# az16/MD_RDM

Measured on AMD Instinct MI355X. Metric: depth-maps/sec NYU 228x304 batch=16 fwd+bwd, higher is better.
Workload: dtype f32 (bf16x6-split 1x1 forward of dense_e2/e3, bf16x3-split gradient GEMMs of dense_e2/e3/e4); 1 GPU; NYU-v2 228x304 batch=16/GPU full train step (fwd+losses+bwd+AdamW), DepthEstimationNet 90.5M params; global_batch=16, parallelism=dp1

## Files before the change

md_rdm_amd/csrc/xsplit.hip:

```cpp
#include <algorithm>
#include <stdlib.h>

#include "rdm_common.h"
#include "elementwise.h"
#include "xsplit.h"
#include "xsplit_dev.h"

namespace rdm {

namespace {

__device__ __forceinline__ bf16x8 tr_frag(const unsigned char* base0, const unsigned char* base1, int imm) {
#if defined(__HIP_DEVICE_COMPILE__)
  typedef s16x4 __attribute__((address_space(3))) * lds_s16x4;
  const s16x4 a = __builtin_amdgcn_ds_read_tr16_b64_v4i16((lds_s16x4)(base0 + imm));
  const s16x4 b = __builtin_amdgcn_ds_read_tr16_b64_v4i16((lds_s16x4)(base1 + imm));
  const s16x8 ab = {a.x, a.y, a.z, a.w, b.x, b.y, b.z, b.w};
  return __builtin_bit_cast(bf16x8, ab);
#else
  return bf16x8{};
#endif
}

struct XsWgradArgs {
// ... 290 lines not shown
          const int idx = b0 + u * 256 + ts, slot = idx / 12, quad = idx - slot * 12;
          if (idx < total4) {
            u32x2 hi, lo;
            split4(v[u][0], v[u][1], v[u][2], v[u][3], hi, lo);
            *reinterpret_cast<u32x2*>(Ahi + (slot + 1) * XD_SLOT + quad * 8) = hi;
            if (NP == 3) *reinterpret_cast<u32x2*>(Alo + (slot + 1) * XD_SLOT + quad * 8) = lo;
          }
        }
      }
      if (ts < 24) *reinterpret_cast<u32x2*>(xs_smem + (ts % 12) * 8 + (ts / 12) * p.plane_bytes) = u32x2{0u, 0u};
      base0 = ((ts & 15) + W + 1 + 1) * XD_SLOT - 32768;
#pragma unroll
      for (int i = 0; i < XD_MT; ++i) {
        const int m = m0 + i * 16 + (ts & 15);
        const bool ok = m < p.M;
        const int b = m / HW, rem = m - b * HW, y = rem / W, x = rem - y * W;
        int v = 0;
#pragma unroll
        for (int tap = 0; tap < 9; ++tap) {
          const int r = tap / 3, q = tap - 3 * r;
          const bool valid = ok && (unsigned)(y + 1 - r) < (unsigned)p.H && (unsigned)(x + 1 - q) < (unsigned)W;
          v |= valid ? (1 << tap) : 0;
        }
        if (i % 3 == 0) vm[i / 3] = v; else vm[i / 3] |= v << (10 * (i % 3));
      }
      __syncthreads();
    }
    const int ct16 = tile * (XD_BN / 16) + 2 * wave;
    if (ct16 * 16 >= p.Cb) continue;
    int ln = lane;
    asm volatile("" : "+v"(ln));
    const int l16 = ln & 15, g = ln >> 4, hi2 = g >> 1;
    const unsigned wv = (unsigned)(ln * 16);
    asm volatile("" : "+v"(base0));
#pragma unroll
    for (int q = 0; q < XD_KSTEPS / 2; ++q) asm volatile("" : "+v"(dpk[q]));
    f32x4 acc[XD_MT][2];
#pragma unroll
    for (int i = 0; i < XD_MT; ++i) { acc[i][0] = f32x4{0.f, 0.f, 0.f, 0.f}; acc[i][1] = f32x4{0.f, 0.f, 0.f, 0.f}; }
    bf16x8 wf[2][2][2];
    auto load_w = [&](int j, bf16x8 (&w)[2][2]) {
#pragma unroll
      for (int t = 0; t < 2; ++t)
#pragma unroll
        for (int pl = 0; pl < (NP == 3 ? 2 : 1); ++pl)
          w[t][pl] = __builtin_bit_cast(bf16x8, __builtin_amdgcn_raw_buffer_load_b128(srdW, (int)(wv + (unsigned)((ct16 + t) * (XD_KSTEPS * 2048))), j * 2048 + pl * 1024, 0));
    };
    const bool t1ok = (ct16 + 1) * 16 < p.Cb;
    f32x4 xv[XD_EA + 1][XD_EC][2];
    f32x4 xs[2] = {{0.f, 0.f, 0.f, 0.f}, {0.f, 0.f, 0.f, 0.f}}, xt[2] = {{0.f, 0.f, 0.f, 0.f}, {0.f, 0.f, 0.f, 0.f}};
    const int c40 = ct16 * 16 + 4 * g;
    int ml = m0 + l16;
    const unsigned vx0 = (unsigned)ml * (unsigned)(p.ldx * 4) + (unsigned)(c40 * 4);
    const int osz = (NP == 1 && p.out_bf16) ? 2 : 4;
    const unsigned vo0 = (unsigned)ml * (unsigned)(p.ldc * osz) + (unsigned)(c40 * osz);
    auto gate_load = [&](int c) {
#pragma unroll
      for (int u = 0; u < XD_EC; ++u)
#pragma unroll
        for (int t = 0; t < 2; ++t) {
          const int i = c * XD_EC + u;
          xv[c % (XD_EA + 1)][u][t] = __builtin_bit_cast(f32x4, __builtin_amdgcn_raw_buffer_load_b128(srdX, (int)(((t == 0 || t1ok) && ml + i * 16 < p.M) ? vx0 + 64u * t : OOB), i * 16 * p.ldx * 4, 0));
        }
    };
    load_w(0, wf[0]);
    bf16x8 gq[2][2];
    auto frag = [&](int j, int i, bf16x8 (&f)[2]) {
      const int dj = (int)((dpk[j >> 1] >> ((j & 1) * 16)) & 0xFFFFu);
      const int tapj = (4 * j) / 6 + (((4 * j) % 6 == 4) ? hi2 : 0);
      const int a = (base0 + i * (16 * XD_SLOT) + dj) & __builtin_amdgcn_sbfe(vm[i / 3], (unsigned)(tapj + 10 * (i % 3)), 1u);
      f[0] = *reinterpret_cast<const bf16x8*>(Ahi + a);
      if (NP == 3) f[1] = *reinterpret_cast<const bf16x8*>(Alo + a);
    };
    frag(0, 0, gq[0]);
#pragma unroll
    for (int j = 0; j < XD_KSTEPS; ++j) {
      if (j + 1 < XD_KSTEPS) load_w(j + 1, wf[(j + 1) & 1]);
      if (MASK && j >= XD_KSTEPS - XD_EK) gate_load(j - (XD_KSTEPS - XD_EK));
#pragma unroll
      for (int i = 0; i < XD_MT; ++i) {
        const int cur = (j * XD_MT + i) & 1;
        if (i + 1 < XD_MT) frag(j, i + 1, gq[cur ^ 1]);
        else if (j + 1 < XD_KSTEPS) frag(j + 1, 0, gq[cur ^ 1]);
        __builtin_amdgcn_sched_barrier(0);
#pragma unroll
        for (int t = 0; t < 2; ++t) {
          if (NP == 3) {
            acc[i][t] = __builtin_amdgcn_mfma_f32_16x16x32_bf16(wf[j & 1][t][1], gq[cur][0], acc[i][t], 0, 0, 0);
            acc[i][t] = __builtin_amdgcn_mfma_f32_16x16x32_bf16(wf[j & 1][t][0], gq[cur][1], acc[i][t], 0, 0, 0);
          }
          acc[i][t] = __builtin_amdgcn_mfma_f32_16x16x32_bf16(wf[j & 1][t][0], gq[cur][0], acc[i][t], 0, 0, 0);
        }
        __builtin_amdgcn_sched_barrier(0);
      }
    }

    f32x4 s0[2] = {{0.f, 0.f, 0.f, 0.f}, {0.f, 0.f, 0.f, 0.f}}, s1[2] = {{0.f, 0.f, 0.f, 0.f}, {0.f, 0.f, 0.f, 0.f}};
    if (MASK) {
#pragma unroll
      for (int t = 0; t < 2; ++t)
        if (t == 0 || t1ok) { xs[t] = *reinterpret_cast<const f32x4*>(p.x_scale + c40 + 16 * t); xt[t] = *reinterpret_cast<const f32x4*>(p.x_shift + c40 + 16 * t); }
#pragma unroll
      for (int c = XD_EK; c < XD_EA; ++c) gate_load(c);
    }
#pragma unroll
    for (int c = 0; c < XD_NCH; ++c) {
      if (MASK && c + XD_EA < XD_NCH) { gate_load(c + XD_EA); __builtin_amdgcn_sched_barrier(0); }
#pragma unroll
      for (int u = 0; u < XD_EC; ++u)
#pragma unroll
        for (int t = 0; t < 2; ++t) {
          const int i = c * XD_EC + u;
          const bool ok = (t == 0 || t1ok) && ml + i * 16 < p.M;
          unsigned char* const orow = reinterpret_cast<unsigned char*>(p.out) + ((long)i * 16 * p.ldc + 16 * t) * osz;
          f32x4 v = acc[i][t];
          if (MASK) {
            const f32x4 x = xv[c % (XD_EA + 1)][u][t];
#pragma unroll
            for (int e = 0; e < 4; ++e) v[e] = fmaf(x[e], xs[t][e], xt[t][e]) > 0.f ? v[e] : 0.f;
            if (ok) { s0[t] += v; s1[t] += v * x; }
          }
          if (NP == 1 && p.out_bf16) {
            const bf16x2 lo2 = {(__bf16)v[0], (__bf16)v[1]}, hi2 = {(__bf16)v[2], (__bf16)v[3]};
            if (ok) *reinterpret_cast<u32x2*>(orow + vo0) = u32x2{__builtin_bit_cast(unsigned, lo2), __builtin_bit_cast(unsigned, hi2)};
          } else if (ok) *reinterpret_cast<f32x4*>(orow + vo0) = v;
        }
    }
    if (MASK) {
      const int sl = 4 * g + l16;
#pragma unroll
      for (int t = 0; t < 2; ++t) {
        const int c4 = ct16 * 16 + 16 * t + sl;
#pragma unroll
        for (int e = 0; e < 4; ++e) {
          float a = s0[t][e], b = s1[t][e];
          a += __shfl_xor(a, 1); b += __shfl_xor(b, 1);
          a += __shfl_xor(a, 2); b += __shfl_xor(b, 2);
          a += __shfl_xor(a, 4); b += __shfl_xor(b, 4);
          a += __shfl_xor(a, 8); b += __shfl_xor(b, 8);
          if (l16 == e) { s0[t][0] = a; s1[t][0] = b; }
        }
        if (l16 < 4 && (t == 0 || t1ok)) {
          atomicAdd(p.stat0 + c4, (double)s0[t][0]);
          atomicAdd(p.stat1 + c4, (double)s1[t][0]);
        }
      }
    }
  }
}


constexpr int X1_MTW_BIG = 5, X1_MTW_SMALL = 2, X1_NTW = 6, X1_BNMAX = 2 * X1_NTW * 16;
constexpr int X1_W_IMG = X1_BNMAX * 64;
constexpr int x1_lds(int mtw) { return 2 * (2 * (4 * mtw * 16 * 64) + 2 * X1_W_IMG); }

struct XsDgrad1Args {
  const float* G; int ldg; int K;
  int g_bf16;
  int g_split;
  int acc;
  const unsigned char* Wp;
  float* out; int ldc;
  const float* X; int ldx; const float* x_scale; const float* x_shift;
  double* stat0; double* stat1;
  int M, C, ksteps;
  int PT;
  int mtiles, ctiles;
  int ct_c0[12], ct_n[12];
  unsigned g_bytes, w_bytes, x_bytes;
};

__global__ __launch_bounds__(256) void k_xs_pack_w1_dgrad(const float* __restrict__ w, int ldw, int K, int C, int ksteps, unsigned char* __restrict__ Wp) {
  const long idx = (long)blockIdx.x * 256 + threadIdx.x;
  const int c = (int)(idx % C);
  const long r1 = idx / C;
  const int ch = (int)(r1 & 3), j = (int)(r1 >> 2);
  if (j >= ksteps) return;
  float v[8];
#pragma unroll
  for (int e = 0; e < 8; ++e) {
    const int k = 32 * j + 8 * ch + e;
    v[e] = k < K ? w[(long)k * ldw + c] : 0.f;
  }
  u32x2 h0, l0, h1, l1;
  split4(v[0], v[1], v[2], v[3], h0, l0);
  split4(v[4], v[5], v[6], v[7], h1, l1);
  const int chs = ch ^ (((c >> 2) & 1) << 1);
  const long plane = (long)ksteps * C * 64;
  unsigned char* dst = Wp + ((long)j * C + c) * 64 + chs * 16;
  *reinterpret_cast<u32x4*>(dst) = u32x4{h0[0], h0[1], h1[0], h1[1]};
  *reinterpret_cast<u32x4*>(dst + plane) = u32x4{l0[0], l0[1], l1[0], l1[1]};
}

template <bool MASK, int NP, int MTW, int D>
__global__ __launch_bounds__(512, 2) void xs_dgrad1x1_kernel(XsDgrad1Args p) {
  constexpr int X1_MTW = MTW, X1_G_IMG = 4 * MTW * 16 * 64, X1_STAGE = 2 * X1_G_IMG + 2 * X1_W_IMG;
  extern __shared__ __attribute__((aligned(1024))) unsigned char x1_smem[];
  const int tid = threadIdx.x, lane = tid & 63, wave = __builtin_amdgcn_readfirstlane(tid >> 6);
  const int l16 = lane & 15, g = lane >> 4;
  const int wc = wave & 1, wp = wave >> 1;
  const unsigned total = gridDim.x, L = blockIdx.x, xq = L & 7u, qq = total >> 3, rr = total & 7u;
  const unsigned item = xq * qq + (xq < rr ? xq : rr) + (L >> 3);
  const int mt = (int)(item / (unsigned)p.ctiles), ctile = (int)(item - (unsigned)mt * (unsigned)p.ctiles);
  const int BM = p.PT * 16, m0 = mt * BM;
  const int nct = p.ct_n[ctile], ct0 = p.ct_c0[ctile], BN = nct * 16;
  const int ntw_max = (nct + 1) >> 1, tw0 = wc * ntw_max, ntw = min(ntw_max, nct - tw0);
  const int npw_max = (p.PT + 3) >> 2, pw0 = wp * npw_max, npw = max(0, min(npw_max, p.PT - pw0));
  const __amdgpu_buffer_rsrc_t srdG = make_srd(p.G, p.g_bytes), srdW = make_srd(p.Wp, p.w_bytes), srdX = make_srd(p.X, p.x_bytes);

  unsigned g_voff[X1_MTW]; unsigned g_lds[X1_MTW]; int g_k[X1_MTW];
#pragma unroll
  for (int u = 0; u < X1_MTW; ++u) {
    const int idx = tid + 512 * u, row = idx >> 3, f4 = idx & 7;
    const bool ok = row < BM && m0 + row < p.M;
    g_k[u] = ok ? 4 * f4 : 0x40000000;
    g_voff[u] = (NP == 1 && p.g_bf16) ? (unsigned)(m0 + row) * (unsigned)(p.ldg * 2) + (unsigned)(f4 * 8)
                                      : (unsigned)(m0 + row) * (unsigned)(p.ldg * 4) + (unsigned)(f4 * 16);
    g_lds[u] = (unsigned)(row * 64 + (((f4 >> 1) ^ (((row >> 2) & 1) << 1)) * 16) + (f4 & 1) * 8);
  }
  const int wpieces = BN * 8;
  const unsigned w_plane = (unsigned)p.ksteps * (unsigned)p.C * 64u;
  f32x4 rg[D][X1_MTW]; u32x4 rw[D][3];
  auto load_slab = [&](int set, int j) {
#pragma unroll
    for (int u = 0; u < X1_MTW; ++u) {
      if (NP == 1 && p.g_bf16) {
        const u32x2 h = __builtin_amdgcn_raw_buffer_load_b64(srdG, (int)((32 * j + g_k[u] < p.K) ? g_voff[u] + (unsigned)(j * 64) : OOB), 0, 0);
        rg[set][u] = f32x4{__uint_as_float(h[0]), __uint_as_float(h[1]), 0.f, 0.f};
      } else {
        rg[set][u] = __builtin_bit_cast(f32x4, __builtin_amdgcn_raw_buffer_load_b128(srdG, (int)((32 * j + g_k[u] < p.K) ? g_voff[u] + (unsigned)(j * 128) : OOB), 0, 0));
      }
    }
#pragma unroll
    for (int u = 0; u < 3; ++u) {
      const int q = tid + 512 * u, pl = q >= BN * 4, r = pl ? q - BN * 4 : q;
      rw[set][u] = __builtin_amdgcn_raw_buffer_load_b128(srdW, (int)((q < wpieces && j < p.ksteps) ? (unsigned)pl * w_plane + ((unsigned)j * (unsigned)p.C + (unsigned)(ct0 * 16)) * 64u + (unsigned)r * 16u : OOB), 0, 0);
    }
  };
  auto store_slab = [&](int set, unsigned char* st) {
#pragma unroll
    for (int u = 0; u < X1_MTW; ++u) {
      if ((tid + 512 * u) >> 3 < BM) {
        u32x2 hi, lo;
        if (NP == 1 && p.g_bf16) hi = u32x2{__float_as_uint(rg[set][u][0]), __float_as_uint(rg[set][u][1])};
        else if (NP == 3 && p.g_split) { hi = u32x2{__float_as_uint(rg[set][u][0]), __float_as_uint(rg[set][u][1])}; lo = u32x2{__float_as_uint(rg[set][u][2]), __float_as_uint(rg[set][u][3])}; }
        else split4(rg[set][u][0], rg[set][u][1], rg[set][u][2], rg[set][u][3], hi, lo);
        *reinterpret_cast<u32x2*>(st + g_lds[u]) = hi;
        if (NP == 3) *reinterpret_cast<u32x2*>(st + X1_G_IMG + g_lds[u]) = lo;
      }
    }
#pragma unroll
    for (int u = 0; u < 3; ++u) {
      const int q = tid + 512 * u, pl = q >= BN * 4, r = pl ? q - BN * 4 : q;
      if (q < wpieces) *reinterpret_cast<u32x4*>(st + 2 * X1_G_IMG + pl * X1_W_IMG + r * 16) = rw[set][u];
    }
  };

  f32x4 acc[X1_MTW][X1_NTW];
#pragma unroll
  for (int i = 0; i < X1_MTW; ++i)
#pragma unroll
    for (int t = 0; t < X1_NTW; ++t) acc[i][t] = f32x4{0.f, 0.f, 0.f, 0.f};
  const unsigned fr = (unsigned)(l16 * 64 + ((g ^ (((l16 >> 2) & 1) << 1)) * 16));

  load_slab(0, 0);
  store_slab(0, x1_smem);
#pragma unroll
  for (int d = 1; d < D; ++d) load_slab(d, d);
  __syncthreads();
  const int ksteps_pad = (p.ksteps + D - 1) / D * D;
  for (int j0 = 0; j0 < ksteps_pad; j0 += D) {
#pragma unroll
    for (int u = 0; u < D; ++u) {
      const int j = j0 + u;
      const bool more = j + 1 < ksteps_pad;
      const unsigned char* const st = x1_smem + (j & 1) * X1_STAGE;
      load_slab(u, j + D);
      bf16x8 gh[X1_MTW], gl[X1_MTW];
#pragma unroll
      for (int i = 0; i < X1_MTW; ++i)
        if (i < npw) {
          gh[i] = *reinterpret_cast<const bf16x8*>(st + (pw0 + i) * 1024 + fr);
          gl[i] = *reinterpret_cast<const bf16x8*>(st + X1_G_IMG + (pw0 + i) * 1024 + fr);
        }
#pragma unroll
      for (int t = 0; t < X1_NTW; ++t)
        if (t < ntw) {
          const bf16x8 wh = *reinterpret_cast<const bf16x8*>(st + 2 * X1_G_IMG + (tw0 + t) * 1024 + fr);
          const bf16x8 wl = *reinterpret_cast<const bf16x8*>(st + 2 * X1_G_IMG + X1_W_IMG + (tw0 + t) * 1024 + fr);
#pragma unroll
          for (int i = 0; i < X1_MTW; ++i)
            if (i < npw) {
              if (NP == 3) {
                acc[i][t] = __builtin_amdgcn_mfma_f32_16x16x32_bf16(wl, gh[i], acc[i][t], 0, 0, 0);
                acc[i][t] = __builtin_amdgcn_mfma_f32_16x16x32_bf16(wh, gl[i], acc[i][t], 0, 0, 0);
              }
              acc[i][t] = __builtin_amdgcn_mfma_f32_16x16x32_bf16(wh, gh[i], acc[i][t], 0, 0, 0);
            }
        }
      if (more) store_slab((u + 1) % D, x1_smem + ((j + 1) & 1) * X1_STAGE);
      __syncthreads();
    }
  }

#pragma unroll
  for (int t = 0; t < X1_NTW; ++t) {
    if (t >= ntw) continue;
    const int c4 = (ct0 + tw0 + t) * 16 + 4 * g;
    const bool cok = c4 < p.C;
    f32x4 xs = {0.f, 0.f, 0.f, 0.f}, xt = {0.f, 0.f, 0.f, 0.f};
    if (MASK && cok) { xs = *reinterpret_cast<const f32x4*>(p.x_scale + c4); xt = *reinterpret_cast<const f32x4*>(p.x_shift + c4); }
    f32x4 s0 = {0.f, 0.f, 0.f, 0.f}, s1 = {0.f, 0.f, 0.f, 0.f};
    const unsigned vx = (unsigned)(m0 + pw0 * 16 + l16) * (unsigned)(p.ldx * 4) + (unsigned)(c4 * 4);
    f32x4 xv[X1_MTW];
    if (MASK) {
#pragma unroll
      for (int i = 0; i < X1_MTW; ++i)
        xv[i] = __builtin_bit_cast(f32x4, __builtin_amdgcn_raw_buffer_load_b128(srdX, (int)((cok && i < npw && m0 + (pw0 + i) * 16 + l16 < p.M) ? vx : OOB), i * 16 * p.ldx * 4, 0));
    }
#pragma unroll
    for (int i = 0; i < X1_MTW; ++i) {
      const int m = m0 + (pw0 + i) * 16 + l16;
      const bool ok = cok && i < npw && m < p.M;
      f32x4 v = acc[i][t];
      if (MASK) {
#pragma unroll
        for (int e = 0; e < 4; ++e) v[e] = fmaf(xv[i][e], xs[e], xt[e]) > 0.f ? v[e] : 0.f;
        if (ok) { s0 += v; s1 += v * xv[i]; }
      }
      if (ok) {
        float* const o = p.out + (long)m * p.ldc + c4;
        if (MASK && p.acc) {
          f32x4 gv = *reinterpret_cast<const f32x4*>(o);
#pragma unroll
          for (int e = 0; e < 4; ++e) gv[e] = fmaf(xs[e], v[e], gv[e]);
          *reinterpret_cast<f32x4*>(o) = gv;
        } else {
          *reinterpret_cast<f32x4*>(o) = v;
        }
      }
    }
    if (MASK) {
#pragma unroll
      for (int e = 0; e < 4; ++e) {
        float a = s0[e], b = s1[e];
        a += __shfl_xor(a, 1); b += __shfl_xor(b, 1);
        a += __shfl_xor(a, 2); b += __shfl_xor(b, 2);
        a += __shfl_xor(a, 4); b += __shfl_xor(b, 4);
        a += __shfl_xor(a, 8); b += __shfl_xor(b, 8);
        if (l16 == e) { s0[0] = a; s1[0] = b; }
      }
      if (l16 < 4 && cok && npw > 0) {
        atomicAdd(p.stat0 + c4 + l16, (double)s0[0]);
        atomicAdd(p.stat1 + c4 + l16, (double)s1[0]);
      }
    }
  }
}


constexpr int XW_D = 2, XW_RING = 256, XW_BC = 64, XW_YPLANE = XW_RING * XW_BC * 2, XW_GPLANE = 32 * 48 * 2;
constexpr int XW_LDS = 2 * XW_YPLANE + 4 * XW_GPLANE;

struct XsWgrad3Args {
  const float* G; int ldg;
  const float* Y; int ldy; int C;
  const float* y_scale; const float* y_shift;
  float* dW; long wtap; int ldw; int N;
  int B, H, W;
  int nslab, split, ahead;
  int g_frame;
  unsigned g_bytes, y_bytes;
};

template <int NP>
__global__ __launch_bounds__(256, 2) void xs_wgrad3x3_kernel(XsWgrad3Args p) {
  __shared__ __attribute__((aligned(1024))) unsigned char smem[XW_LDS];
  unsigned char* const Yhi = smem;
  unsigned char* const Ylo = smem + XW_YPLANE;
  unsigned char* const Gb = smem + 2 * XW_YPLANE;
  const int tid = threadIdx.x, lane = tid & 63, wave = __builtin_amdgcn_readfirstlane(tid >> 6);
  const int l16 = lane & 15, g = lane >> 4;
  const int grp = tid >> 4, kq = l16 >> 2, jq = l16 & 3;
  const int Wp = p.W + 2, PP = (p.H + 2) * Wp, U = p.B * PP;
  const int c0 = blockIdx.x * XW_BC;
  const int per = (p.nslab + p.split - 1) / p.split;
  const int s_begin = blockIdx.y * per, s_end = min(p.nslab, s_begin + per);
  if (s_begin >= s_end) return;
  const __amdgpu_buffer_rsrc_t srdG = make_srd(p.G, p.g_bytes), srdY = make_srd(p.Y, p.y_bytes);
  const bool bnrelu = p.y_scale != nullptr;

  const int yc = c0 + 16 * (grp & 3) + 4 * jq;
  const bool ycok = yc < p.C;
  f32x4 ysc = {1.f, 1.f, 1.f, 1.f}, ysh = {0.f, 0.f, 0.f, 0.f};
  if (bnrelu && ycok) { ysc = *reinterpret_cast<const f32x4*>(p.y_scale + yc); ysh = *reinterpret_cast<const f32x4*>(p.y_shift + yc); }
  const float rPP = 1.0f / (float)PP, rWp = 1.0f / (float)Wp;
  auto pix_off = [&](int u, int ld, int col, bool colok) -> unsigned {
    const int b = (int)(((float)u + 0.5f) * rPP), rem = u - b * PP, yp = (int)(((float)rem + 0.5f) * rWp), xp = rem - yp * Wp;
    const bool ok = u >= 0 && u < U && colok && yp >= 1 && yp <= p.H && xp >= 1 && xp <= p.W;
    return ok ? (unsigned)((b * p.H + yp - 1) * p.W + xp - 1) * (unsigned)(ld * 4) + (unsigned)(col * 4) : OOB;
  };
  auto y_lds = [&](int s, int it) -> unsigned {
    const int row = ((s & 7) << 5) + 4 * ((grp >> 2) + 4 * it) + kq;
    const int rb = row >> 3, pr = (row & 7) ^ ((rb & 1) << 2);
    return (unsigned)(256 * (rb * 4 + (grp & 3)) + 32 * pr + 8 * jq);
  };
  f32x4 ry[XW_D][2]; unsigned yin = 0u;
  auto load_y = [&](int set, int s) {
#pragma unroll
    for (int it = 0; it < 2; ++it) {
      const unsigned off = pix_off(s * 32 + 4 * ((grp >> 2) + 4 * it) + kq, p.ldy, yc, ycok);
      ry[set][it] = __builtin_bit_cast(f32x4, __builtin_amdgcn_raw_buffer_load_b128(srdY, (int)off, 0, 0));
      yin = (yin & ~(1u << (2 * set + it))) | (off != OOB ? 1u << (2 * set + it) : 0u);
    }
  };
  auto store_y = [&](int set, int s) {
#pragma unroll
    for (int it = 0; it < 2; ++it) {
      f32x4 v = ry[set][it];
      if (bnrelu) {
        const float top = (yin >> (2 * set + it)) & 1u ? __builtin_inff() : 0.f;
#pragma unroll
        for (int e = 0; e < 4; ++e) v[e] = __builtin_amdgcn_fmed3f(fmaf(v[e], ysc[e], ysh[e]), 0.f, top);
      }
      u32x2 hi, lo;
      split4(v[0], v[1], v[2], v[3], hi, lo);
      const unsigned a = y_lds(s, it);
      *reinterpret_cast<u32x2*>(Yhi + a) = hi;
      if (NP == 3) *reinterpret_cast<u32x2*>(Ylo + a) = lo;
    }
  };
  f32x4 rgv[XW_D][2];
  auto load_g = [&](int set, int s) {
#pragma unroll
    for (int it = 0; it < 2; ++it) {
      const int pi = grp + 16 * it, rg = pi / 3, ct = pi - 3 * rg;
      unsigned off;
      if (NP == 3 && p.g_frame) off = (pi < 24 && s >= 0) ? (unsigned)(s * 32 + 4 * rg + kq) * 192u + (unsigned)((16 * ct + 4 * jq) * 4) : OOB;
      else off = pi < 24 ? pix_off(s * 32 + 4 * rg + kq, p.ldg, 16 * ct + 4 * jq, 16 * ct + 4 * jq < p.N) : OOB;
      rgv[set][it] = __builtin_bit_cast(f32x4, __builtin_amdgcn_raw_buffer_load_b128(srdG, (int)off, 0, 0));
    }
  };
  auto store_g = [&](int set, int s) {
    unsigned char* const gb = Gb + (s & 1) * (2 * XW_GPLANE);
#pragma unroll
    for (int it = 0; it < 2; ++it) {
      const int pi = grp + 16 * it, rg = pi / 3, ct = pi - 3 * rg;
      if (pi < 24) {
        u32x2 hi, lo;
        if (NP == 3 && p.g_frame) { hi = u32x2{__float_as_uint(rgv[set][it][0]), __float_as_uint(rgv[set][it][1])}; lo = u32x2{__float_as_uint(rgv[set][it][2]), __float_as_uint(rgv[set][it][3])}; }
        else split4(rgv[set][it][0], rgv[set][it][1], rgv[set][it][2], rgv[set][it][3], hi, lo);
        const int row = 4 * rg + kq, rb = row >> 3, pr = (row & 7) ^ ((rb & 1) << 2);
        const unsigned a = (unsigned)(256 * (rb * 3 + ct) + 32 * pr + 8 * jq);
        *reinterpret_cast<u32x2*>(gb + a) = hi;
        if (NP == 3) *reinterpret_cast<u32x2*>(gb + XW_GPLANE + a) = lo;
// ... 277 lines not shown

}

bool xs_wgrad1x1_supported(const WgradArgs& a) {
  const bool one = a.g.KH == 1 && a.g.KW == 1 && a.g.SH == 1 && a.g.SW == 1 && a.g.PH == 0 && a.g.PW == 0 && a.g.H == a.g.Ho && a.g.W == a.g.Wo;
  return one && a.C % 48 == 0 && a.C >= 96 && a.C <= 12 * 192 && a.N % 4 == 0;
}

int launch_xs_wgrad1x1(const WgradArgs& a, hipStream_t s) {
  RDM_CHECK_ARG(xs_wgrad1x1_supported(a), "split-precision 1x1 wgrad: needs a 1x1 / stride 1 convolution with 96 <= C (%d) <= 2304, C a multiple of 48, N (%d) of 4", a.C, a.N);
  RDM_CHECK_ARG(a.ldg % 4 == 0 && a.ldx % 4 == 0 && ((uintptr_t)a.G & 15) == 0 && ((uintptr_t)a.Xs & 15) == 0, "split-precision 1x1 wgrad: strides multiples of 4 floats, operands 16-byte aligned");
  const long M = (long)a.g.B * a.g.Ho * a.g.Wo;
  RDM_CHECK_ARG(!a.g_bf16 || a.xsplit == 1, "1x1 wgrad: bf16 gradient rows exist in the one-product (mixed-precision) form only");
  const long gb = ((M - 1) * a.ldg + a.N) * (a.g_bf16 ? 2 : 4), xb = ((M - 1) * a.ldx + a.C) * 4;
  if (gb >= 0xFFFFFFFFL || xb >= 0xFFFFFFFFL) { set_error("split-precision 1x1 wgrad: operand extent >= 4 GiB is not supported by the 32-bit buffer addressing"); return RDM_ERR_UNSUPPORTED; }
  RDM_CHECK_ARG((!a.g_split && !a.x_split) || a.xsplit != 1, "1x1 wgrad: split rows are operands of the three-product form");
  RDM_CHECK_ARG(!a.x_split || (a.x_scale == nullptr && a.x_shift == nullptr), "1x1 wgrad: split activation rows are already activated (no BatchNorm prologue)");
  XsWgradArgs k{};
  k.g_bf16 = a.g_bf16; k.g_split = a.g_split; k.x_split = a.x_split;
  k.G = a.G; k.ldg = a.ldg; k.N = a.N; k.X = a.Xs; k.ldx = a.ldx; k.C = a.C; k.x_scale = a.x_scale; k.x_shift = a.x_shift;
  k.dW = a.dW; k.ldw = a.ldw; k.M = (int)M; k.g_bytes = (unsigned)gb; k.x_bytes = (unsigned)xb;
  const int units = a.C / 48, nct = (units + 3) / 4;
  int c0 = 0;
  for (int t = 0; t < nct; ++t) {
    const int u = units / nct + (t < units % nct ? 1 : 0);
    k.ct_c0[t] = c0; k.ct_nt[t] = 3 * u;
    c0 += 48 * u;
  }
  k.n_ctiles = nct;
  const long tiles = (long)nct * cdiv(a.N, XS_BM), kslabs = (M + XS_BK - 1) / XS_BK;
  const long tiles128 = (long)nct * cdiv(a.N, 128);
  const long split128 = tiles128 > 512 ? pick_split_k(tiles128, kslabs / 2, 256 * 2) : std::max<long>(1, std::min<long>(512 / tiles128, kslabs / 16));
  long split = 1;
  if (split128 > 1) split = std::max<long>(2, tiles > 256 ? pick_split_k(tiles, kslabs / 2, 256) : std::min<long>(256 / tiles, kslabs / 16));
  if (a.split_k > 0) split = a.split_k;
  k.split_k = (int)std::min<long>(split, kslabs);
  void* prof = profile_begin(s, 2.0 * (double)M * a.N * a.C, 13);
  RDM_CENSUS("xs_wgrad1x1_kernel/x%d/%s/%s%s", a.xsplit == 1 ? 1 : 3, a.x_scale ? "bn1" : "bn0", k.split_k > 1 ? "splitK" : "split1", a.g_split && a.x_split ? "/rowsGX" : a.g_split ? "/rowsG" : a.x_split ? "/rowsX" : "");
  if (a.xsplit == 1) hipLaunchKernelGGL(xs_wgrad1x1_kernel<1>, dim3((unsigned)(tiles * k.split_k)), dim3(512), 0, s, k);
  else hipLaunchKernelGGL(xs_wgrad1x1_kernel<3>, dim3((unsigned)(tiles * k.split_k)), dim3(512), 0, s, k);
  profile_end(prof, s);
  RDM_LAUNCH_OK();
  return 0;
}

size_t xs_dgrad3x3_workspace_bytes(int Cb) { return (size_t)(Cb / 16) * XD_KSTEPS * 2048; }

static int xs_dgrad3_lds_bytes(int W) {
  const int nslots = 1 + XD_BM + 2 * (W + 1);
  const int plane = (nslots * XD_SLOT + 1023) & ~1023;
  return 2 * plane;
}

bool xs_dgrad3x3_supported(const FwdArgs& a) {
  const ConvGeom& g = a.g;
  return g.KH == 3 && g.KW == 3 && g.SH == 1 && g.SW == 1 && g.PH == 1 && g.PW == 1 && g.H == g.Ho && g.W == g.Wo && g.dir == -1 && a.C == 48 &&
         a.N % 16 == 0 && a.N >= 16 && xs_dgrad3_lds_bytes(g.W) <= 156 * 1024 && (g.W + 2) * XD_SLOT < 32768 && a.bias == nullptr && !a.accumulate && !a.add_out;
}

int launch_xs_pack_w3_dgrad(const float* w, long wtap, int ldw, int Cb, void* ws, hipStream_t s) {
  const long threads = (long)(Cb / 16) * XD_KSTEPS * 64;
  hipLaunchKernelGGL(k_xs_pack_w3_dgrad, dim3((unsigned)cdiv(threads, 256)), dim3(256), 0, s, w, wtap, ldw, Cb, static_cast<unsigned char*>(ws));
  RDM_LAUNCH_OK();
  return 0;
}

int launch_xs_dgrad3x3(const FwdArgs& a, Epilogue epi, void* ws, size_t ws_bytes, hipStream_t s, int np, bool prepacked) {
  RDM_CHECK_ARG(xs_dgrad3x3_supported(a), "split-precision 3x3 dgrad: needs a 3x3 / stride 1 / pad 1 convolution with 48 gradient channels, N (%d) a multiple of 16, W (%d) <= 339", a.N, a.g.W);
  RDM_CHECK_ARG(epi == EPI_STORE || epi == EPI_MASK_STATS, "split-precision 3x3 dgrad: plain or gate + statistics epilogue only");
  RDM_CHECK_ARG(a.lda % 4 == 0 && a.ldc % 4 == 0 && a.ldw % 4 == 0 && ((uintptr_t)a.A & 15) == 0 && ((uintptr_t)a.out & 15) == 0, "split-precision 3x3 dgrad: strides multiples of 4 floats, tensors 16-byte aligned");
  RDM_CHECK_ARG(epi != EPI_MASK_STATS || (a.X && a.x_scale && a.x_shift && a.stat0 && a.stat1 && a.ldx % 4 == 0 && ((uintptr_t)a.X & 15) == 0), "split-precision 3x3 dgrad: the gate needs X, scale, shift and both statistics");
  RDM_CHECK_ARG(ws != nullptr && ((uintptr_t)ws & 15) == 0 && ws_bytes >= xs_dgrad3x3_workspace_bytes(a.N), "split-precision 3x3 dgrad: workspace too small or misaligned (%zu < %zu)", ws_bytes, xs_dgrad3x3_workspace_bytes(a.N));
  const long M = a.M;
  const long gb = ((M - 1) * a.lda + 48) * 4, ob = ((M - 1) * a.ldc + a.N) * 4, xb = a.X ? ((M - 1) * a.ldx + a.N) * 4 : 16;
  if (gb >= 0xFFFFFFFFL || ob >= 0xFFFFFFFFL || xb >= 0xFFFFFFFFL) { set_error("split-precision 3x3 dgrad: operand extent >= 4 GiB is not supported by the 32-bit buffer addressing"); return RDM_ERR_UNSUPPORTED; }
  const int Cb = a.N;
  if (!prepacked) { if (int prc = launch_xs_pack_w3_dgrad(a.Wt, a.wtap, a.ldw, Cb, ws, s)) return prc; }
  XsDgrad3Args k{};
  k.G = a.A; k.ldg = a.lda; k.Wf = static_cast<const unsigned char*>(ws); k.out = a.out; k.ldc = a.ldc;
  k.X = a.X; k.ldx = a.ldx; k.x_scale = a.x_scale; k.x_shift = a.x_shift; k.stat0 = a.stat0; k.stat1 = a.stat1;
  RDM_CHECK_ARG(!a.out_bf16 || np == 1, "3x3 dgrad: bf16 output rows exist in the one-product (mixed-precision) form only");
  k.out_bf16 = a.out_bf16;
  k.B = a.g.B; k.H = a.g.H; k.W = a.g.W; k.M = (int)M; k.Cb = Cb;
  k.nslots = 1 + XD_BM + 2 * (a.g.W + 1);
  k.plane_bytes = (k.nslots * XD_SLOT + 1023) & ~1023;
  k.mtiles = cdiv(M, XD_BM); k.ctiles = cdiv(Cb, XD_BN);
  k.g_bytes = (unsigned)gb; k.w_bytes = (unsigned)xs_dgrad3x3_workspace_bytes(Cb); k.x_bytes = (unsigned)xb; k.o_bytes = (unsigned)ob;
  const int lds = xs_dgrad3_lds_bytes(a.g.W);
  const long items = (long)k.mtiles * k.ctiles;
  const long slots = 256L * (lds <= 80 * 1024 ? 2 : 1);
  void* prof = profile_begin(s, 2.0 * (double)M * Cb * 432.0, 14);
  RDM_CENSUS("xs_dgrad3x3_kernel/x%d/%s", np == 1 ? 1 : 3, epi == EPI_MASK_STATS ? "MASK_STATS" : "STORE");
  const dim3 grid((unsigned)std::min(items, slots));
#define RDM_XS_D3(MASK_, NP_) do { \
    RDM_HIP_OK(hipFuncSetAttribute(reinterpret_cast<const void*>(&xs_dgrad3x3_kernel<MASK_, NP_>), hipFuncAttributeMaxDynamicSharedMemorySize, lds)); \
    hipLaunchKernelGGL((xs_dgrad3x3_kernel<MASK_, NP_>), grid, dim3(256), lds, s, k); } while (0)
  if (epi == EPI_MASK_STATS) { if (np == 1) RDM_XS_D3(true, 1); else RDM_XS_D3(true, 3); }
  else { if (np == 1) RDM_XS_D3(false, 1); else RDM_XS_D3(false, 3); }
#undef RDM_XS_D3
  profile_end(prof, s);
  RDM_LAUNCH_OK();
  return 0;
}

size_t xs_dgrad1x1_workspace_bytes(int K, int C) { return (size_t)2 * ((K + 31) / 32) * C * 64; }

bool xs_dgrad1x1_supported(const FwdArgs& a) {
  const ConvGeom& g = a.g;
  const bool one = g.KH == 1 && g.KW == 1 && g.SH == 1 && g.SW == 1 && g.PH == 0 && g.PW == 0 && g.H == g.Ho && g.W == g.Wo;
  return one && a.N % 16 == 0 && a.N >= 16 && a.N <= 12 * X1_BNMAX && a.C % 4 == 0 && a.C >= 32 && a.bias == nullptr && !a.accumulate && !a.add_out;
}

int launch_xs_pack_w1_dgrad(const float* w, int ldw, int K, int C, void* ws, hipStream_t s) {
  const int ksteps = (K + 31) / 32;
  const long threads = (long)ksteps * 4 * C;
  hipLaunchKernelGGL(k_xs_pack_w1_dgrad, dim3((unsigned)cdiv(threads, 256)), dim3(256), 0, s, w, ldw, K, C, ksteps, static_cast<unsigned char*>(ws));
  RDM_LAUNCH_OK();
  return 0;
}

int launch_xs_dgrad1x1(const FwdArgs& a, Epilogue epi, void* ws, size_t ws_bytes, hipStream_t s, int np, bool prepacked) {
  RDM_CHECK_ARG(xs_dgrad1x1_supported(a), "split-precision 1x1 dgrad: needs a 1x1 / stride 1 convolution, 16 <= N (%d) <= %d a multiple of 16, C (%d) a multiple of 4", a.N, 12 * X1_BNMAX, a.C);
  RDM_CHECK_ARG(epi == EPI_STORE || epi == EPI_MASK_STATS, "split-precision 1x1 dgrad: plain or gate + statistics epilogue only");
  RDM_CHECK_ARG(a.lda % 4 == 0 && a.ldc % 4 == 0 && a.ldw % 4 == 0 && ((uintptr_t)a.A & 15) == 0 && ((uintptr_t)a.out & 15) == 0, "split-precision 1x1 dgrad: strides multiples of 4 floats, tensors 16-byte aligned");
  RDM_CHECK_ARG(epi != EPI_MASK_STATS || (a.X && a.x_scale && a.x_shift && a.stat0 && a.stat1 && a.ldx % 4 == 0 && ((uintptr_t)a.X & 15) == 0), "split-precision 1x1 dgrad: the gate needs X, scale, shift and both statistics");
  const int K = a.C, C = a.N, ksteps = (K + 31) / 32;
  RDM_CHECK_ARG(ws != nullptr && ((uintptr_t)ws & 15) == 0 && ws_bytes >= xs_dgrad1x1_workspace_bytes(K, C), "split-precision 1x1 dgrad: workspace too small or misaligned (%zu < %zu)", ws_bytes, xs_dgrad1x1_workspace_bytes(K, C));
  const long M = a.M;
  RDM_CHECK_ARG(!a.a_bf16 || np == 1, "1x1 dgrad: bf16 gradient rows exist in the one-product (mixed-precision) form only");
  const long gb = ((M - 1) * a.lda + K) * (a.a_bf16 ? 2 : 4), xb = a.X ? ((M - 1) * a.ldx + C) * 4 : 16;
  if (gb >= 0xFFFFFFFFL || xb >= 0xFFFFFFFFL) { set_error("split-precision 1x1 dgrad: operand extent >= 4 GiB is not supported by the 32-bit buffer addressing"); return RDM_ERR_UNSUPPORTED; }
  if (!prepacked) { if (int prc = launch_xs_pack_w1_dgrad(a.Wt, a.ldw, K, C, ws, s)) return prc; }
  XsDgrad1Args k{};
  RDM_CHECK_ARG(!a.acc_scaled || epi == EPI_MASK_STATS, "1x1 dgrad: the accumulating epilogue comes with the gate");
  k.acc = a.acc_scaled;
  RDM_CHECK_ARG(!a.a_split || np != 1, "1x1 dgrad: split rows are the operand of the three-product form");
  k.g_split = a.a_split;
  k.G = a.A; k.ldg = a.lda; k.K = K; k.g_bf16 = a.a_bf16; k.Wp = static_cast<const unsigned char*>(ws); k.out = a.out; k.ldc = a.ldc;
  k.X = a.X; k.ldx = a.ldx; k.x_scale = a.x_scale; k.x_shift = a.x_shift; k.stat0 = a.stat0; k.stat1 = a.stat1;
  k.M = (int)M; k.C = C; k.ksteps = ksteps;
  const int nct = C / 16, ctiles = (nct + 2 * X1_NTW - 1) / (2 * X1_NTW);
  int c0 = 0;
  for (int t = 0; t < ctiles; ++t) { k.ct_c0[t] = c0; k.ct_n[t] = nct / ctiles + (t < nct % ctiles ? 1 : 0); c0 += k.ct_n[t]; }
  k.ctiles = ctiles;
  const bool small = M <= 8192;
  const int mtw = small ? X1_MTW_SMALL : X1_MTW_BIG;
  int best_pt = 1; long best_cost = -1;
  for (int pt = 1; pt <= 4 * mtw; ++pt) {
    const long items = (long)cdiv(M, 16 * pt) * ctiles, rounds = (items + 255) / 256;
    const long cost = rounds * (pt * 16 + 24);
    if (best_cost < 0 || cost < best_cost) { best_cost = cost; best_pt = pt; }
  }
  k.PT = best_pt; k.mtiles = cdiv(M, 16 * best_pt);
  k.g_bytes = (unsigned)gb; k.w_bytes = (unsigned)xs_dgrad1x1_workspace_bytes(K, C); k.x_bytes = (unsigned)xb;
  void* prof = profile_begin(s, 2.0 * (double)M * C * K, 16);
  RDM_CENSUS("xs_dgrad1x1_kernel/x%d/%s/%s%s", np == 1 ? 1 : 3, small ? "px128" : "px320", epi == EPI_MASK_STATS ? "MASK_STATS" : "STORE", a.a_split ? "/rowsG" : "");
  const dim3 grid((unsigned)(k.mtiles * k.ctiles));
#define RDM_XS_D1B(MASK_, NP_, MTW_, D_) do { \
    RDM_HIP_OK(hipFuncSetAttribute(reinterpret_cast<const void*>(&xs_dgrad1x1_kernel<MASK_, NP_, MTW_, D_>), hipFuncAttributeMaxDynamicSharedMemorySize, x1_lds(MTW_))); \
    hipLaunchKernelGGL((xs_dgrad1x1_kernel<MASK_, NP_, MTW_, D_>), grid, dim3(512), x1_lds(MTW_), s, k); } while (0)
#define RDM_XS_D1(MASK_, NP_) do { if (small) RDM_XS_D1B(MASK_, NP_, X1_MTW_SMALL, 1); else RDM_XS_D1B(MASK_, NP_, X1_MTW_BIG, 1); } while (0)
  if (epi == EPI_MASK_STATS) { if (np == 1) RDM_XS_D1(true, 1); else RDM_XS_D1(true, 3); }
  else { if (np == 1) RDM_XS_D1(false, 1); else RDM_XS_D1(false, 3); }
#undef RDM_XS_D1
#undef RDM_XS_D1B
  profile_end(prof, s);
  RDM_LAUNCH_OK();
  return 0;
}

__global__ __launch_bounds__(256) void k_frame_split_rows(const float* __restrict__ G, int ldg, int N, int B, int H, int W, int upad, u32x4* __restrict__ dst) {
  const int Wp = W + 2, PP = (H + 2) * Wp;
  const float rPP = 1.0f / (float)PP, rWp = 1.0f / (float)Wp;
  const int t = threadIdx.x, pl = (int)((unsigned)t * 2731u >> 15), q = t - pl * 12;
  if (t >= 252) return;
  for (int u = blockIdx.x * 21 + pl; u < upad; u += gridDim.x * 21) {
    const int b = (int)(((float)u + 0.5f) * rPP), rem = u - b * PP, yp = (int)(((float)rem + 0.5f) * rWp), xp = rem - yp * Wp;
    f32x4 v = {0.f, 0.f, 0.f, 0.f};
    if (b < B && yp >= 1 && yp <= H && xp >= 1 && xp <= W && 4 * q < N) v = *reinterpret_cast<const f32x4*>(G + ((long)(b * H + yp - 1) * W + xp - 1) * ldg + 4 * q);
    dst[(long)u * 12 + q] = split_row4(v[0], v[1], v[2], v[3]);
  }
}

size_t xs_frame_rows_bytes(int B, int H, int W) { return (size_t)(((long)B * (H + 2) * (W + 2) + 31) / 32 * 32) * 192; }

int launch_frame_split_rows(const float* G, int ldg, int N, int B, int H, int W, void* dst, hipStream_t s) {
  RDM_CHECK_ARG(N >= 4 && N <= 48 && N % 4 == 0 && ldg % 4 == 0 && ((uintptr_t)G & 15) == 0 && ((uintptr_t)dst & 15) == 0, "frame_split_rows: N (%d) a multiple of 4 up to 48, ldg a multiple of 4, operands 16-byte aligned", N);
  const long upad = ((long)B * (H + 2) * (W + 2) + 31) / 32 * 32;
  RDM_CHECK_ARG(upad < (1L << 21), "frame_split_rows: %ld padded positions (the float-reciprocal frame arithmetic is exact below 2^21)", upad);
  hipLaunchKernelGGL(k_frame_split_rows, dim3((unsigned)std::min<long>(cdiv(upad, 21), 256 * 16)), dim3(256), 0, s, G, ldg, N, B, H, W, (int)upad, static_cast<u32x4*>(dst));
  RDM_LAUNCH_OK();
  return 0;
}

bool xs_wgrad3x3_supported(const WgradArgs& a) {
  const ConvGeom& g = a.g;
  return g.KH == 3 && g.KW == 3 && g.SH == 1 && g.SW == 1 && g.PH == 1 && g.PW == 1 && g.H == g.Ho && g.W == g.Wo && g.dir == 1 && a.N <= 48 && a.N % 4 == 0 &&
         a.C % 4 == 0 && a.C >= 16 && (g.W + 3 + 31) / 32 <= 3;
}

int launch_xs_wgrad3x3(const WgradArgs& a, hipStream_t s) {
  RDM_CHECK_ARG(xs_wgrad3x3_supported(a), "split-precision 3x3 wgrad: needs a 3x3 / stride 1 / pad 1 convolution with N (%d) <= 48, N and C (%d) multiples of 4, W (%d) <= 93", a.N, a.C, a.g.W);
  RDM_CHECK_ARG(a.ldg % 4 == 0 && a.ldx % 4 == 0 && a.ldw % 4 == 0 && ((uintptr_t)a.G & 15) == 0 && ((uintptr_t)a.Xs & 15) == 0, "split-precision 3x3 wgrad: strides multiples of 4 floats, operands 16-byte aligned");
  const long M = (long)a.g.B * a.g.H * a.g.W;
  RDM_CHECK_ARG(!a.g_frame || a.xsplit != 1, "3x3 wgrad: the frame image is an operand of the three-product form");
  const long gb = a.g_frame ? (long)xs_frame_rows_bytes(a.g.B, a.g.H, a.g.W) : ((M - 1) * a.ldg + a.N) * 4, yb = ((M - 1) * a.ldx + a.C) * 4;
  if (gb >= 0xFFFFFFFFL || yb >= 0xFFFFFFFFL) { set_error("split-precision 3x3 wgrad: operand extent >= 4 GiB is not supported by the 32-bit buffer addressing"); return RDM_ERR_UNSUPPORTED; }
  XsWgrad3Args k{};
  k.g_frame = a.g_frame;
  k.G = a.G; k.ldg = a.ldg; k.Y = a.Xs; k.ldy = a.ldx; k.C = a.C; k.y_scale = a.x_scale; k.y_shift = a.x_shift;
  k.dW = a.dW; k.wtap = a.wtap; k.ldw = a.ldw; k.N = a.N; k.B = a.g.B; k.H = a.g.H; k.W = a.g.W;
  const long U = (long)a.g.B * (a.g.H + 2) * (a.g.W + 2);
  k.nslab = (int)((U + 31) / 32);
  k.ahead = (a.g.W + 3 + 31) / 32;
  const int cblocks = cdiv(a.C, XW_BC);
  int best = 1; double best_cost = 1e30;
  const int max_split = a.split_k > 0 ? a.split_k : 64;
  for (int sp = a.split_k > 0 ? a.split_k : 1; sp <= max_split && sp <= std::max(1, k.nslab / 8); ++sp) {
    const long rounds = ((long)cblocks * sp + 511) / 512;
    const double cost = rounds * ((k.nslab + sp - 1) / sp + 2.0 * k.ahead + 3.0 + 8.0);
    if (cost < best_cost - 1e-9) { best_cost = cost; best = sp; }
  }
  k.split = best;
  k.g_bytes = (unsigned)gb; k.y_bytes = (unsigned)yb;
  void* prof = profile_begin(s, 2.0 * (double)M * a.N * 9.0 * a.C, 15);
  RDM_CENSUS("xs_wgrad3x3_kernel/x%d/%s%s", a.xsplit == 1 ? 1 : 3, a.x_scale ? "bn1" : "bn0", a.g_frame ? "/frameG" : "");
  if (a.xsplit == 1) hipLaunchKernelGGL(xs_wgrad3x3_kernel<1>, dim3((unsigned)cblocks, (unsigned)k.split), dim3(256), 0, s, k);
  else hipLaunchKernelGGL(xs_wgrad3x3_kernel<3>, dim3((unsigned)cblocks, (unsigned)k.split), dim3(256), 0, s, k);
  profile_end(prof, s);
  RDM_LAUNCH_OK();
  return 0;
}

size_t xs_fwd1x1_workspace_bytes(int K, int N) { return (size_t)3 * ((K + 31) / 32) * N * 64; }

bool xs_fwd1x1_supported(const FwdArgs& a) {
  const ConvGeom& g = a.g;
  const bool one = g.KH == 1 && g.KW == 1 && g.SH == 1 && g.SW == 1 && g.PH == 0 && g.PW == 0 && g.H == g.Ho && g.W == g.Wo && g.dir == 1;
  return one && a.N % 16 == 0 && a.N >= 16 && a.C % 4 == 0 && a.C >= 4 && a.bias == nullptr && !a.accumulate && !a.add_out && a.a_sum == nullptr;
}

int launch_xs_pack_w1_fwd(const float* w, int ldw, int N, int K, void* ws, hipStream_t s) {
  const int ksteps = (K + 31) / 32;
  const long threads = (long)ksteps * N * 4;
  hipLaunchKernelGGL(k_xs_pack_w1_fwd, dim3((unsigned)cdiv(threads, 256)), dim3(256), 0, s, w, ldw, N, K, ksteps, static_cast<unsigned char*>(ws));
  RDM_LAUNCH_OK();
  return 0;
}

int launch_xs_fwd1x1(const FwdArgs& a, Epilogue epi, void* ws, size_t ws_bytes, hipStream_t s, int np, bool prepacked) {
  RDM_CHECK_ARG(xs_fwd1x1_supported(a), "split-precision 1x1 forward: needs a 1x1 / stride 1 convolution, N (%d) a multiple of 16, C (%d) a multiple of 4, no bias / accumulation", a.N, a.C);
  RDM_CHECK_ARG(epi == EPI_STORE || epi == EPI_STORE_STATS, "split-precision 1x1 forward: plain or statistics epilogue only");
  RDM_CHECK_ARG(a.lda % 4 == 0 && a.ldc % 4 == 0 && a.ldw % 4 == 0 && ((uintptr_t)a.A & 15) == 0 && ((uintptr_t)a.out & 15) == 0, "split-precision 1x1 forward: strides multiples of 4 floats, tensors 16-byte aligned");
  RDM_CHECK_ARG((a.a_scale == nullptr) == (a.a_shift == nullptr) && (a.a_scale == nullptr || (((uintptr_t)a.a_scale | (uintptr_t)a.a_shift) & 15) == 0), "split-precision 1x1 forward: scale and shift go together, 16-byte aligned");
  RDM_CHECK_ARG(epi != EPI_STORE_STATS || (a.stat0 && a.stat1), "split-precision 1x1 forward: the statistics epilogue needs both sums");
  const int K = a.C, N = a.N, ksteps = (K + 31) / 32;
  RDM_CHECK_ARG(ws != nullptr && ((uintptr_t)ws & 15) == 0 && ws_bytes >= xs_fwd1x1_workspace_bytes(K, N), "split-precision 1x1 forward: workspace too small or misaligned (%zu < %zu)", ws_bytes, xs_fwd1x1_workspace_bytes(K, N));
  const long M = a.M;
  const long xb = ((M - 1) * a.lda + K) * 4;
  if (xb >= 0xFFFFFFFFL) { set_error("split-precision 1x1 forward: operand extent >= 4 GiB is not supported by the 32-bit buffer addressing"); return RDM_ERR_UNSUPPORTED; }
  if (!prepacked) { if (int prc = launch_xs_pack_w1_fwd(a.Wt, a.ldw, N, K, ws, s)) return prc; }
  XsFwd1Args k{};
  k.X = a.A; k.ldx = a.lda; k.K = K; k.x_scale = a.a_scale; k.x_shift = a.a_shift; k.Wp = static_cast<const unsigned char*>(ws);
  k.out = a.out; k.ldc = a.ldc; k.stat0 = a.stat0; k.stat1 = a.stat1; k.M = (int)M; k.N = N; k.ksteps = ksteps;
  k.ctiles = cdiv(N / 16, 2 * XF_NTW);
  constexpr int mtw = 4, slots = 256;
  int best_pt = 1; long best_cost = -1;
  for (int pt = 1; pt <= 4 * mtw; ++pt) {
    const long items = (long)cdiv(M, 16 * pt) * k.ctiles, rounds = (items + slots - 1) / slots;
    const long cost = rounds * (pt * 16 + 24);
    if (best_cost < 0 || cost < best_cost) { best_cost = cost; best_pt = pt; }
  }
  k.PT = best_pt; k.mtiles = cdiv(M, 16 * best_pt);
  k.x_bytes = (unsigned)xb; k.w_bytes = (unsigned)xs_fwd1x1_workspace_bytes(K, N);
  void* prof = profile_begin(s, 2.0 * (double)M * N * K, 17);
  RDM_CENSUS("xs_fwd1x1_kernel/x%d/%s/%s", np == 1 ? 1 : 6, a.a_scale ? "bn1" : "bn0", epi == EPI_STORE_STATS ? "STORE_STATS" : "STORE");
  const dim3 grid((unsigned)(k.mtiles * k.ctiles));
#define RDM_XS_F1M(STATS_, NP_, MTW_) do { \
    RDM_HIP_OK(hipFuncSetAttribute(reinterpret_cast<const void*>(&xs_fwd1x1_kernel<STATS_, NP_, MTW_>), hipFuncAttributeMaxDynamicSharedMemorySize, xf_lds(MTW_))); \
    hipLaunchKernelGGL((xs_fwd1x1_kernel<STATS_, NP_, MTW_>), grid, dim3(512), xf_lds(MTW_), s, k); } while (0)
#define RDM_XS_F1(STATS_, NP_) RDM_XS_F1M(STATS_, NP_, 4)
  if (epi == EPI_STORE_STATS) { if (np == 1) RDM_XS_F1(true, 1); else RDM_XS_F1(true, 6); }
  else { if (np == 1) RDM_XS_F1(false, 1); else RDM_XS_F1(false, 6); }
#undef RDM_XS_F1
#undef RDM_XS_F1M
  profile_end(prof, s);
  RDM_LAUNCH_OK();
  return 0;
}

}
```

Baseline: 348.2 images/s.

## Add LDS-DMA ring pipeline for small-M 1x1 dgrad kernel

For the small-M variant of the 1x1 dgrad split-bf16 kernel, this adds a separate k-loop. It uses a ring of LDS stages: three when the grid fits in one wave of blocks, two otherwise. Weights, and pre-split G rows when present, are loaded straight into LDS with buffer-to-LDS DMA, and G is stored in a new swizzled interleaved hi/lo layout. The aim is to hide global-load latency behind MFMA work and remove the register staging round trip. The cost is more LDS per block, which may reduce occupancy, plus hand-written waitcnt and barrier sequencing.

New measurement: 346.3 images/s. No clear change (-0.5%).

```diff
diff --git a/md_rdm_amd/csrc/xsplit.hip b/md_rdm_amd/csrc/xsplit.hip
--- a/md_rdm_amd/csrc/xsplit.hip
+++ b/md_rdm_amd/csrc/xsplit.hip
@@ -466,7 +466,9 @@
 
 constexpr int X1_MTW_BIG = 5, X1_MTW_SMALL = 2, X1_NTW = 6, X1_BNMAX = 2 * X1_NTW * 16;
 constexpr int X1_W_IMG = X1_BNMAX * 64;
-constexpr int x1_lds(int mtw) { return 2 * (2 * (4 * mtw * 16 * 64) + 2 * X1_W_IMG); }
+constexpr int X1_SMALL_STAGES = 3;
+constexpr int x1_lds(int mtw, int stages = 2) { return stages * (2 * (4 * mtw * 16 * 64) + 2 * X1_W_IMG); }
+constexpr int x1_lds_max(int mtw) { return x1_lds(mtw, mtw == X1_MTW_SMALL ? X1_SMALL_STAGES : 2); }
 
 struct XsDgrad1Args {
   const float* G; int ldg; int K;
@@ -479,6 +481,7 @@
   double* stat0; double* stat1;
   int M, C, ksteps;
   int PT;
+  int stages;
   int mtiles, ctiles;
   int ct_c0[12], ct_n[12];
   unsigned g_bytes, w_bytes, x_bytes;
@@ -522,6 +525,115 @@
   const int npw_max = (p.PT + 3) >> 2, pw0 = wp * npw_max, npw = max(0, min(npw_max, p.PT - pw0));
   const __amdgpu_buffer_rsrc_t srdG = make_srd(p.G, p.g_bytes), srdW = make_srd(p.Wp, p.w_bytes), srdX = make_srd(p.X, p.x_bytes);
 
+  f32x4 acc[X1_MTW][X1_NTW];
+#pragma unroll
+  for (int i = 0; i < X1_MTW; ++i)
+#pragma unroll
+    for (int t = 0; t < X1_NTW; ++t) acc[i][t] = f32x4{0.f, 0.f, 0.f, 0.f};
+  const unsigned fr = (unsigned)(l16 * 64 + ((g ^ (((l16 >> 2) & 1) << 1)) * 16));
+
+  if constexpr (MTW == X1_MTW_SMALL) {
+    constexpr int NPC = X1_MTW + 3;
+    auto gsw = [](int r) { return (r & 6) | (((r >> 2) ^ (r >> 3)) & 1); };
+    unsigned g_voff[X1_MTW]; int g_k[X1_MTW];
+#pragma unroll
+    for (int u = 0; u < X1_MTW; ++u) {
+      const int idx = tid + 512 * u, row = idx >> 3, q = (idx & 7) ^ gsw(row);
+      const bool ok = row < BM && m0 + row < p.M;
+      g_k[u] = ok ? 4 * q : 0x40000000;
+      g_voff[u] = (NP == 1 && p.g_bf16) ? (unsigned)(m0 + row) * (unsigned)(p.ldg * 2) + (unsigned)(q * 8)
+                                        : (unsigned)(m0 + row) * (unsigned)(p.ldg * 4) + (unsigned)(q * 16);
+    }
+    unsigned w_voff[3];
+#pragma unroll
+    for (int u = 0; u < 3; ++u) {
+      const int q = wave + 8 * u, pl = q >= nct, t = q - pl * nct;
+      w_voff[u] = q < 2 * nct ? (unsigned)pl * ((unsigned)p.ksteps * (unsigned)p.C * 64u) + (unsigned)(ct0 * 16) * 64u + (unsigned)(t * 1024 + lane * 16) : OOB;
+    }
+    auto issue_w = [&](int j, unsigned so) {
+#pragma unroll
+      for (int u = 0; u < 3; ++u) lds_dma16(srdW, j < p.ksteps ? w_voff[u] : OOB, (unsigned)j * (unsigned)p.C * 64u, x1_smem + so + 2 * X1_G_IMG + (wave + 8 * u) * 1024);
+    };
+    auto issue_g = [&](int j, unsigned so) {
+#pragma unroll
+      for (int u = 0; u < X1_MTW; ++u) lds_dma16(srdG, (32 * j + g_k[u] < p.K) ? g_voff[u] : OOB, (unsigned)j * 128u, x1_smem + so + (wave + 8 * u) * 1024);
+    };
+    f32x4 rg[X1_MTW];
+    auto load_g = [&](int j) {
+#pragma unroll
+      for (int u = 0; u < X1_MTW; ++u) {
+        if (NP == 1 && p.g_bf16) {
+          const u32x2 h = __builtin_amdgcn_raw_buffer_load_b64(srdG, (int)((32 * j + g_k[u] < p.K) ? g_voff[u] + (unsigned)(j * 64) : OOB), 0, 0);
+          rg[u] = f32x4{__uint_as_float(h[0]), __uint_as_float(h[1]), 0.f, 0.f};
+        } else {
+          rg[u] = __builtin_bit_cast(f32x4, __builtin_amdgcn_raw_buffer_load_b128(srdG, (int)((32 * j + g_k[u] < p.K) ? g_voff[u] + (unsigned)(j * 128) : OOB), 0, 0));
+        }
+      }
+    };
+    auto store_g = [&](unsigned so) {
+#pragma unroll
+      for (int u = 0; u < X1_MTW; ++u) {
+        const int idx = tid + 512 * u;
+        if (idx >> 3 < BM) {
+          u32x2 hi, lo;
+          if (NP == 1 && p.g_bf16) hi = u32x2{__float_as_uint(rg[u][0]), __float_as_uint(rg[u][1])};
+          else split4(rg[u][0], rg[u][1], rg[u][2], rg[u][3], hi, lo);
+          if (NP == 3) *reinterpret_cast<u32x4*>(x1_smem + so + idx * 16) = u32x4{hi[0], hi[1], lo[0], lo[1]};
+          else *reinterpret_cast<u32x2*>(x1_smem + so + idx * 16) = hi;
+        }
+      }
+    };
+    const unsigned ga = (unsigned)(l16 * 128 + (((2 * g) ^ gsw(l16)) * 16)), gb = (unsigned)(l16 * 128 + (((2 * g + 1) ^ gsw(l16)) * 16));
+    auto mma = [&](unsigned so) {
+      const unsigned char* const st = x1_smem + so;
+      bf16x8 gh[X1_MTW], gl[X1_MTW];
+#pragma unroll
+      for (int i = 0; i < X1_MTW; ++i)
+        if (i < npw) {
+          const u32x4 a = *reinterpret_cast<const u32x4*>(st + (pw0 + i) * 2048 + ga), b = *reinterpret_cast<const u32x4*>(st + (pw0 + i) * 2048 + gb);
+          gh[i] = __builtin_bit_cast(bf16x8, u32x4{a[0], a[1], b[0], b[1]});
+          gl[i] = __builtin_bit_cast(bf16x8, u32x4{a[2], a[3], b[2], b[3]});
+        }
+#pragma unroll
+      for (int t = 0; t < X1_NTW; ++t)
+        if (t < ntw) {
+          const bf16x8 wh = *reinterpret_cast<const bf16x8*>(st + 2 * X1_G_IMG + (tw0 + t) * 1024 + fr);
+          const bf16x8 wl = *reinterpret_cast<const bf16x8*>(st + 2 * X1_G_IMG + (nct + tw0 + t) * 1024 + fr);
+#pragma unroll
+          for (int i = 0; i < X1_MTW; ++i)
+            if (i < npw) {
+              if (NP == 3) {
+                acc[i][t] = __builtin_amdgcn_mfma_f32_16x16x32_bf16(wl, gh[i], acc[i][t], 0, 0, 0);
+                acc[i][t] = __builtin_amdgcn_mfma_f32_16x16x32_bf16(wh, gl[i], acc[i][t], 0, 0, 0);
+              }
+              acc[i][t] = __builtin_amdgcn_mfma_f32_16x16x32_bf16(wh, gh[i], acc[i][t], 0, 0, 0);
+            }
+        }
+    };
+    auto kloop = [&](auto dma) {
+      constexpr bool DMA = decltype(dma)::value;
+      const bool deep = p.stages == X1_SMALL_STAGES;
+      const unsigned ring = (unsigned)p.stages * X1_STAGE;
+      const int ahead = p.stages - 1;
+      unsigned sa = 0u, sc = ring - X1_STAGE;
+      if (DMA) { issue_g(0, 0u); issue_w(0, 0u); if (deep) { issue_g(1, X1_STAGE); issue_w(1, X1_STAGE); } }
+      else { load_g(0); issue_w(0, 0u); store_g(0u); if (deep) { load_g(1); issue_w(1, X1_STAGE); store_g(X1_STAGE); } }
+      for (int j = 0; j < p.ksteps; ++j) {
+        if (deep) asm volatile("s_waitcnt vmcnt(%0) lgkmcnt(0)" ::"n"(NPC) : "memory");
+        else asm volatile("s_waitcnt vmcnt(0) lgkmcnt(0)" ::: "memory");
+        __builtin_amdgcn_s_barrier();
+        asm volatile("" ::: "memory");
+        if (DMA) { issue_g(j + ahead, sc); issue_w(j + ahead, sc); }
+        else { load_g(j + ahead); issue_w(j + ahead, sc); }
+        mma(sa);
+        if (!DMA) store_g(sc);
+        sa = sa + X1_STAGE == ring ? 0u : sa + X1_STAGE;
+        sc = sc + X1_STAGE == ring ? 0u : sc + X1_STAGE;
+      }
+      asm volatile("s_waitcnt vmcnt(0)" ::: "memory");
+    };
+    if (NP == 3 && p.g_split) kloop(std::true_type{}); else kloop(std::false_type{});
+  } else {
   unsigned g_voff[X1_MTW]; unsigned g_lds[X1_MTW]; int g_k[X1_MTW];
 #pragma unroll
   for (int u = 0; u < X1_MTW; ++u) {
@@ -570,13 +682,6 @@
     }
   };
 
-  f32x4 acc[X1_MTW][X1_NTW];
-#pragma unroll
-  for (int i = 0; i < X1_MTW; ++i)
-#pragma unroll
-    for (int t = 0; t < X1_NTW; ++t) acc[i][t] = f32x4{0.f, 0.f, 0.f, 0.f};
-  const unsigned fr = (unsigned)(l16 * 64 + ((g ^ (((l16 >> 2) & 1) << 1)) * 16));
-
   load_slab(0, 0);
   store_slab(0, x1_smem);
 #pragma unroll
@@ -615,6 +720,7 @@
       if (more) store_slab((u + 1) % D, x1_smem + ((j + 1) & 1) * X1_STAGE);
       __syncthreads();
     }
+  }
   }
 
 #pragma unroll
@@ -1198,13 +1304,14 @@
     if (best_cost < 0 || cost < best_cost) { best_cost = cost; best_pt = pt; }
   }
   k.PT = best_pt; k.mtiles = cdiv(M, 16 * best_pt);
+  k.stages = small && (long)k.mtiles * ctiles <= 256 ? X1_SMALL_STAGES : 2;
   k.g_bytes = (unsigned)gb; k.w_bytes = (unsigned)xs_dgrad1x1_workspace_bytes(K, C); k.x_bytes = (unsigned)xb;
   void* prof = profile_begin(s, 2.0 * (double)M * C * K, 16);
   RDM_CENSUS("xs_dgrad1x1_kernel/x%d/%s/%s%s", np == 1 ? 1 : 3, small ? "px128" : "px320", epi == EPI_MASK_STATS ? "MASK_STATS" : "STORE", a.a_split ? "/rowsG" : "");
   const dim3 grid((unsigned)(k.mtiles * k.ctiles));
 #define RDM_XS_D1B(MASK_, NP_, MTW_, D_) do { \
-    RDM_HIP_OK(hipFuncSetAttribute(reinterpret_cast<const void*>(&xs_dgrad1x1_kernel<MASK_, NP_, MTW_, D_>), hipFuncAttributeMaxDynamicSharedMemorySize, x1_lds(MTW_))); \
-    hipLaunchKernelGGL((xs_dgrad1x1_kernel<MASK_, NP_, MTW_, D_>), grid, dim3(512), x1_lds(MTW_), s, k); } while (0)
+    RDM_HIP_OK(hipFuncSetAttribute(reinterpret_cast<const void*>(&xs_dgrad1x1_kernel<MASK_, NP_, MTW_, D_>), hipFuncAttributeMaxDynamicSharedMemorySize, x1_lds_max(MTW_))); \
+    hipLaunchKernelGGL((xs_dgrad1x1_kernel<MASK_, NP_, MTW_, D_>), grid, dim3(512), x1_lds(MTW_, k.stages), s, k); } while (0)
 #define RDM_XS_D1(MASK_, NP_) do { if (small) RDM_XS_D1B(MASK_, NP_, X1_MTW_SMALL, 1); else RDM_XS_D1B(MASK_, NP_, X1_MTW_BIG, 1); } while (0)
   if (epi == EPI_MASK_STATS) { if (np == 1) RDM_XS_D1(true, 1); else RDM_XS_D1(true, 3); }
   else { if (np == 1) RDM_XS_D1(false, 1); else RDM_XS_D1(false, 3); }
```
